# Owen-Liuyuxuan/FSNet

Measured on AMD Instinct MI355X. Metric: training samples/sec (3-frame triplets) at 192x640, ResNet-18 depth+pose, higher is better.
Workload: dtype bf16; 1 GPU; KITTI Eigen-Zhou-shaped synthetic triplets, ResNet-18 depth+pose, 192x640, bf16, batch 12/GPU, full step (fwd+loss+bwd+clip35+Adam); inputs HBM-resident, no H2D in the timed region; global_batch=12, parallelism=dp1, encoder_pass=two chains (depth and pose encoder on two streams), autotune_steps=0, hipgraph_replays=574

## Files before the change

fsnet_amd/csrc/pool_upsample.hip:

```cpp
#include "common.h"
#include "fsnet_hip_internal.h"
#include <algorithm>

namespace {

struct FsPoolPair { const void* in1; void* out1; uint8_t* idx1; const void* add1; int n0; };

template <typename T>
__global__ __launch_bounds__(256) void maxpool_fwd_kernel(const T* __restrict__ x, T* __restrict__ y,
                                                          uint8_t* __restrict__ idx, int N, int H, int W, int C,
                                                          int Ho, int Wo, FsPoolPair pr) {
  constexpr int VN = VecN<T>::N;
  const int CG = C / VN;
  const long total = (long)N * Ho * Wo * CG;
  for (long i = (long)blockIdx.x * 256 + threadIdx.x; i < total; i += (long)gridDim.x * 256) {
    int cg = (int)(i % CG); long m = i / CG;
    int wo = (int)(m % Wo); long q = m / Wo; int ho = (int)(q % Ho); long n = q / Ho;
    const T* xs = x; T* ys = y; uint8_t* is = idx;
    if (n >= pr.n0) {
      n -= pr.n0; m -= (long)pr.n0 * Ho * Wo;
      xs = reinterpret_cast<const T*>(pr.in1); ys = reinterpret_cast<T*>(pr.out1); is = pr.idx1;
    }
    float best[VN];
    int bi[VN];
#pragma unroll
    for (int j = 0; j < VN; ++j) { best[j] = -INFINITY; bi[j] = 0; }
    bool first = true;
    for (int r = 0; r < 3; ++r) {
      int h = ho * 2 - 1 + r;
      if ((unsigned)h >= (unsigned)H) continue;
      for (int s = 0; s < 3; ++s) {
        int w = wo * 2 - 1 + s;
        if ((unsigned)w >= (unsigned)W) continue;
        float v[VN];
        loadv<T>(xs + ((n * H + h) * W + w) * C + cg * VN, v);
#pragma unroll
        for (int j = 0; j < VN; ++j)
          if (first || v[j] > best[j]) { best[j] = v[j]; bi[j] = r * 3 + s; }
        first = false;
      }
    }
    storev<T>(ys + m * C + cg * VN, best);
#pragma unroll
    for (int k = 0; k < VN / 4; ++k) {
      uint32_t packed = (uint32_t)bi[4 * k] | ((uint32_t)bi[4 * k + 1] << 8) | ((uint32_t)bi[4 * k + 2] << 16) |
                        ((uint32_t)bi[4 * k + 3] << 24);
      reinterpret_cast<uint32_t*>(is + m * C + cg * VN)[k] = packed;
    }
  }
}

template <typename T>
__global__ __launch_bounds__(256) void maxpool_bwd_kernel(const T* __restrict__ dy, const uint8_t* __restrict__ idx,
                                                          const T* __restrict__ addend, T* __restrict__ dx, int N,
// ... 14 lines not shown
#pragma unroll
    for (int j = 0; j < VN; ++j) acc[j] = 0.f;
    if (ads) loadv<T>(ads + m * C + cg * VN, acc);
    for (int ho = (h - 1 + 1) / 2; ho <= (h + 1) / 2; ++ho) {
      if (ho < 0 || ho >= Ho) continue;
      int r = h - (ho * 2 - 1);
      if (r < 0 || r > 2) continue;
      for (int wo = w / 2; wo <= (w + 1) / 2; ++wo) {
        if (wo < 0 || wo >= Wo) continue;
        int s = w - (wo * 2 - 1);
        if (s < 0 || s > 2) continue;
        long mo = (n * Ho + ho) * Wo + wo;
        uint32_t packed[VN / 4];
#pragma unroll
        for (int k = 0; k < VN / 4; ++k) packed[k] = reinterpret_cast<const uint32_t*>(is + mo * C + cg * VN)[k];
        float g[VN];
        loadv<T>(dys + mo * C + cg * VN, g);
        int code = r * 3 + s;
#pragma unroll
        for (int j = 0; j < VN; ++j)
          if ((int)((packed[j >> 2] >> (8 * (j & 3))) & 0xff) == code) acc[j] += g[j];
      }
    }
    storev<T>(dxs + m * C + cg * VN, acc);
  }
}

template <typename T, int V> __device__ inline void ldc(const T* p, float* v) {
  if constexpr (V == 8) loadv<T>(p, v); else load4<T>(p, v);
}
template <typename T, int V> __device__ inline void stc(T* p, const float* v) {
  if constexpr (V == 8) storev<T>(p, v); else store4<T>(p, v);
}

template <typename T, int V>
__global__ __launch_bounds__(256) void upcat_pad_fwd_kernel(const T* __restrict__ a, const T* __restrict__ b,
                                                            T* __restrict__ out, int N, int h, int w, int Ca,
                                                            int Cb) {
  const int H = 2 * h, W = 2 * w, Hp = H + 2, Wp = W + 2, C = Ca + Cb, CG = C / V;
  const long total = (long)N * Hp * Wp * CG;
  for (long i = (long)blockIdx.x * 256 + threadIdx.x; i < total; i += (long)gridDim.x * 256) {
    int cg = (int)(i % CG); long m = i / CG;
    int wp = (int)(m % Wp); long q = m / Wp; int hp = (int)(q % Hp); long n = q / Hp;
    int hi = min(max(hp - 1, 0), H - 1), wi = min(max(wp - 1, 0), W - 1);
    int c = cg * V;
    float v[V];
    if (c < Ca) ldc<T, V>(a + ((n * h + (hi >> 1)) * w + (wi >> 1)) * Ca + c, v);
    else ldc<T, V>(b + ((n * H + hi) * W + wi) * Cb + (c - Ca), v);
    stc<T, V>(out + m * C + c, v);
  }
}

template <typename T, int V>
__device__ inline void fold_load(const T* dpad, long n, int hi, int wi, int H, int W, int C, int c, float* g) {
  const int Hp = H + 2, Wp = W + 2;
  int hs[2] = {hi + 1, 0}, ws[2] = {wi + 1, 0};
  int nh = 1, nw = 1;
  if (hi == 0) { hs[1] = 0; nh = 2; } else if (hi == H - 1) { hs[1] = H + 1; nh = 2; }
  if (wi == 0) { ws[1] = 0; nw = 2; } else if (wi == W - 1) { ws[1] = W + 1; nw = 2; }
#pragma unroll
  for (int j = 0; j < V; ++j) g[j] = 0.f;
  for (int x = 0; x < nh; ++x)
    for (int y = 0; y < nw; ++y) {
      float t[V];
      ldc<T, V>(dpad + ((n * Hp + hs[x]) * Wp + ws[y]) * C + c, t);
#pragma unroll
      for (int j = 0; j < V; ++j) g[j] += t[j];
    }
}

template <typename T, int V>
__global__ __launch_bounds__(256) void upcat_pad_bwd_kernel(const T* __restrict__ dpad, T* __restrict__ da,
                                                            T* __restrict__ db, int N, int h, int w, int Ca,
                                                            int Cb) {
  const int H = 2 * h, W = 2 * w, C = Ca + Cb;
  const int CGa = Ca / V, CGb = Cb / V;
  const long ta = (long)N * h * w * CGa, tb = (long)N * H * W * CGb;
  for (long i = (long)blockIdx.x * 256 + threadIdx.x; i < ta + tb; i += (long)gridDim.x * 256) {
    if (i < ta) {
      int cg = (int)(i % CGa); long m = i / CGa;
      int x = (int)(m % w); long q = m / w; int y = (int)(q % h); long n = q / h;
      float acc[V];
#pragma unroll
      for (int j = 0; j < V; ++j) acc[j] = 0.f;
      for (int dy = 0; dy < 2; ++dy)
        for (int dx = 0; dx < 2; ++dx) {
          float g[V];
          fold_load<T, V>(dpad, n, 2 * y + dy, 2 * x + dx, H, W, C, cg * V, g);
#pragma unroll
          for (int j = 0; j < V; ++j) acc[j] += g[j];
        }
      stc<T, V>(da + m * Ca + cg * V, acc);
    } else {
      long k = i - ta;
      int cg = (int)(k % CGb); long m = k / CGb;
      int x = (int)(m % W); long q = m / W; int y = (int)(q % H); long n = q / H;
      float g[V];
      fold_load<T, V>(dpad, n, y, x, H, W, C, Ca + cg * V, g);
      stc<T, V>(db + m * Cb + cg * V, g);
    }
  }
}

template <typename T> __device__ __forceinline__ float round_to(float v);
template <> __device__ __forceinline__ float round_to<float>(float v) { return v; }
template <> __device__ __forceinline__ float round_to<bf16>(float v) { return bf16_bits_to_f(f_to_bf16_bits(v)); }

template <typename T, int V>
__global__ __launch_bounds__(256) void upcat_pad_bwd_bn_kernel(const T* __restrict__ dpad, T* __restrict__ da,
                                                               T* __restrict__ db, int N, int h, int w, int Ca, int Cb,
                                                               const T* __restrict__ yact, const T* __restrict__ xraw,
                                                               const float* __restrict__ mean,
                                                               const float* __restrict__ invstd, double* __restrict__ sums,
                                                               const int nA) {
  const int H = 2 * h, W = 2 * w, C = Ca + Cb;
  const int CGa = Ca / V, CGb = Cb / V;
  if ((int)blockIdx.x >= nA) {
    const long tb = (long)N * H * W * CGb;
    const int bx = (int)blockIdx.x - nA, nB = (int)gridDim.x - nA;
    for (long k = (long)bx * 256 + threadIdx.x; k < tb; k += (long)nB * 256) {
      int cg = (int)(k % CGb); long m = k / CGb;
      int x = (int)(m % W); long q = m / W; int y = (int)(q % H); long n = q / H;
      float g[V];
      fold_load<T, V>(dpad, n, y, x, H, W, C, Ca + cg * V, g);
      stc<T, V>(db + m * Cb + cg * V, g);
    }
    return;
  }
  __shared__ float red[2][V][256];
  const int cg = threadIdx.x % CGa, c = cg * V;
  float mu[V], is[V], s1[V], s2[V];
#pragma unroll
  for (int j = 0; j < V; ++j) { mu[j] = mean[c + j]; is[j] = invstd[c + j]; s1[j] = 0.f; s2[j] = 0.f; }
  const long ta = (long)N * h * w * CGa;
  for (long i = (long)blockIdx.x * 256 + threadIdx.x; i < ta; i += (long)nA * 256) {
    long m = i / CGa;
    int x = (int)(m % w); long q = m / w; int y = (int)(q % h); long n = q / h;
    float acc[V], yy[V], xr[V];
    ldc<T, V>(yact + m * Ca + c, yy);
    ldc<T, V>(xraw + m * Ca + c, xr);
#pragma unroll
    for (int j = 0; j < V; ++j) acc[j] = 0.f;
    for (int dy = 0; dy < 2; ++dy)
      for (int dx = 0; dx < 2; ++dx) {
        float g[V];
        fold_load<T, V>(dpad, n, 2 * y + dy, 2 * x + dx, H, W, C, c, g);
#pragma unroll
        for (int j = 0; j < V; ++j) acc[j] += g[j];
      }
#pragma unroll
    for (int j = 0; j < V; ++j) {
      const float g = yy[j] > 0.f ? round_to<T>(acc[j]) : 0.f;
      acc[j] = g;
      s1[j] += g; s2[j] += g * (xr[j] - mu[j]) * is[j];
    }
    stc<T, V>(da + m * Ca + c, acc);
  }
#pragma unroll
  for (int j = 0; j < V; ++j) { red[0][j][threadIdx.x] = s1[j]; red[1][j][threadIdx.x] = s2[j]; }
  __syncthreads();
  const int PL = 256 / CGa;
  for (int t = threadIdx.x; t < CGa * 2 * V; t += 256) {
    const int g2 = t % CGa, kj = t / CGa, kind = kj / V, j = kj % V;
    float a = 0.f;
    for (int k = 0; k < PL; ++k) a += red[kind][j][k * CGa + g2];
    double* sl = sums + (long)(blockIdx.x % FS_STAT_SLOTS) * 2 * Ca;
    atomicAdd(sl + kind * Ca + g2 * V + j, (double)a);
  }
}

template <typename T, int VL>
__device__ __forceinline__ void channel_sum_body(const T* __restrict__ x, float* __restrict__ out, long M, int C, int Creal,
                                                 int CGB, int bx, int by, int gx) {
  __shared__ float red[VL][256];
  const int CG = C / VL;
  const int PL = 256 / CGB;
  const int cgl = threadIdx.x % CGB, pl = threadIdx.x / CGB;
  const int cg = by * CGB + cgl;
  float s[VL];
#pragma unroll
  for (int j = 0; j < VL; ++j) s[j] = 0.f;
  auto ld = [&](long m, float* v) {
    if constexpr (VL == 4) load4<T>(x + m * C + cg * 4, v);
    else loadv<T>(x + m * C + cg * VL, v);
  };
  if (cg < CG) {
    const long stride = (long)gx * PL;
    long m = (long)bx * PL + pl;
    for (; m + 3 * stride < M; m += 4 * stride) {
      float v0[VL], v1[VL], v2[VL], v3[VL];
      ld(m, v0); ld(m + stride, v1); ld(m + 2 * stride, v2); ld(m + 3 * stride, v3);
#pragma unroll
      for (int j = 0; j < VL; ++j) s[j] += (v0[j] + v1[j]) + (v2[j] + v3[j]);
// ... 77 lines not shown
  if (!dy || !dx || !idx || C % vn != 0 || N <= 0) return FS_EINVAL;
  if (dy1 && (!dx1 || !idx1 || N1 <= 0)) return FS_EINVAL;
  if (!dy1) N1 = 0;
  hipStream_t st = reinterpret_cast<hipStream_t>(stream);
  int Ho = (H + 2 - 3) / 2 + 1, Wo = (W + 2 - 3) / 2 + 1;
  const FsPoolPair pr{dy1, dx1, const_cast<uint8_t*>(idx1), addend1, dy1 ? N : 0x7fffffff};
  dim3 grid(grid_for((long)(N + N1) * H * W * (C / vn)));
  if (dtype == FS_DTYPE_BF16)
    hipLaunchKernelGGL(maxpool_bwd_kernel<bf16>, grid, dim3(256), 0, st, (const bf16*)dy, idx, (const bf16*)addend, (bf16*)dx, N + N1, H, W, C, Ho, Wo, pr);
  else if (dtype == FS_DTYPE_F32)
    hipLaunchKernelGGL(maxpool_bwd_kernel<float>, grid, dim3(256), 0, st, (const float*)dy, idx, (const float*)addend, (float*)dx, N + N1, H, W, C, Ho, Wo, pr);
  else return FS_EINVAL;
  return fs_launch_status();
}

extern "C" int fs_maxpool_bwd(const void* dy, const uint8_t* idx, const void* addend, void* dx, int N, int H, int W,
                              int C, int dtype, void* stream) {
  return fs_maxpool_bwd2(dy, idx, addend, dx, N, nullptr, nullptr, nullptr, nullptr, 0, H, W, C, dtype, stream);
}

extern "C" int fs_upcat_pad_fwd(const void* a, const void* b, void* out, int N, int h, int w, int Ca, int Cb,
                                int dtype, void* stream) {
  if (!a || !out || (Cb > 0 && !b) || Ca % 4 != 0 || Cb % 4 != 0) return FS_EINVAL;
  hipStream_t st = reinterpret_cast<hipStream_t>(stream);
  const bool wide = dtype == FS_DTYPE_BF16 && Ca % 8 == 0 && Cb % 8 == 0;
  dim3 grid(grid_for((long)N * (2 * h + 2) * (2 * w + 2) * ((Ca + Cb) / (wide ? 8 : 4))));
  if (wide)
    hipLaunchKernelGGL((upcat_pad_fwd_kernel<bf16, 8>), grid, dim3(256), 0, st, (const bf16*)a, (const bf16*)b, (bf16*)out, N, h, w, Ca, Cb);
  else if (dtype == FS_DTYPE_BF16)
    hipLaunchKernelGGL((upcat_pad_fwd_kernel<bf16, 4>), grid, dim3(256), 0, st, (const bf16*)a, (const bf16*)b, (bf16*)out, N, h, w, Ca, Cb);
  else if (dtype == FS_DTYPE_F32)
    hipLaunchKernelGGL((upcat_pad_fwd_kernel<float, 4>), grid, dim3(256), 0, st, (const float*)a, (const float*)b, (float*)out, N, h, w, Ca, Cb);
  else return FS_EINVAL;
  return fs_launch_status();
}

extern "C" int fs_upcat_pad_bwd(const void* dpad, void* da, void* db, int N, int h, int w, int Ca, int Cb, int dtype,
                                void* stream) {
  if (!dpad || !da || (Cb > 0 && !db) || Ca % 4 != 0 || Cb % 4 != 0) return FS_EINVAL;
  hipStream_t st = reinterpret_cast<hipStream_t>(stream);
  const bool wide = dtype == FS_DTYPE_BF16 && Ca % 8 == 0 && Cb % 8 == 0;
  const int V = wide ? 8 : 4;
  dim3 grid(grid_for((long)N * h * w * (Ca / V) + (long)N * 4 * h * w * (Cb / V)));
  if (wide)
    hipLaunchKernelGGL((upcat_pad_bwd_kernel<bf16, 8>), grid, dim3(256), 0, st, (const bf16*)dpad, (bf16*)da, (bf16*)db, N, h, w, Ca, Cb);
  else if (dtype == FS_DTYPE_BF16)
    hipLaunchKernelGGL((upcat_pad_bwd_kernel<bf16, 4>), grid, dim3(256), 0, st, (const bf16*)dpad, (bf16*)da, (bf16*)db, N, h, w, Ca, Cb);
  else if (dtype == FS_DTYPE_F32)
    hipLaunchKernelGGL((upcat_pad_bwd_kernel<float, 4>), grid, dim3(256), 0, st, (const float*)dpad, (float*)da, (float*)db, N, h, w, Ca, Cb);
  else return FS_EINVAL;
  return fs_launch_status();
}

extern "C" int fs_upcat_pad_bwd_bn(const void* dpad, void* da, void* db, int N, int h, int w, int Ca, int Cb, const void* y,
                                   const void* x, const float* mean, const float* invstd, double* sums, int dtype,
                                   void* stream) {
  if (!dpad || !da || (Cb > 0 && !db) || !y || !x || !mean || !invstd || !sums || Ca % 4 != 0 || Cb % 4 != 0 || Ca <= 0)
    return FS_EINVAL;
  hipStream_t st = reinterpret_cast<hipStream_t>(stream);
  const bool wide = dtype == FS_DTYPE_BF16 && Ca % 8 == 0 && Cb % 8 == 0;
  const int V = wide ? 8 : 4;
  const int CGa = Ca / V;
  if (CGa > 256 || 256 % CGa != 0) return FS_EINVAL;
  const long ta = (long)N * h * w * CGa, tb = (long)N * 4 * h * w * (Cb / V);
  const int nA = (int)std::max<long>(1, std::min<long>((ta + 511) / 512, 512));
  const int nB = Cb > 0 ? grid_for(tb) : 0;
  dim3 grid(nA + nB);
  if (wide)
    hipLaunchKernelGGL((upcat_pad_bwd_bn_kernel<bf16, 8>), grid, dim3(256), 0, st, (const bf16*)dpad, (bf16*)da, (bf16*)db, N, h, w, Ca, Cb,
                       (const bf16*)y, (const bf16*)x, mean, invstd, sums, nA);
  else if (dtype == FS_DTYPE_BF16)
    hipLaunchKernelGGL((upcat_pad_bwd_bn_kernel<bf16, 4>), grid, dim3(256), 0, st, (const bf16*)dpad, (bf16*)da, (bf16*)db, N, h, w, Ca, Cb,
                       (const bf16*)y, (const bf16*)x, mean, invstd, sums, nA);
  else if (dtype == FS_DTYPE_F32)
    hipLaunchKernelGGL((upcat_pad_bwd_bn_kernel<float, 4>), grid, dim3(256), 0, st, (const float*)dpad, (float*)da, (float*)db, N, h, w, Ca, Cb,
                       (const float*)y, (const float*)x, mean, invstd, sums, nA);
  else return FS_EINVAL;
  return fs_launch_status();
}

extern "C" int fs_channel_sum_multi(const void* const* x, float* const* out, const int64_t* M, const int32_t* C,
                                    const int32_t* Creal, int n, int dtype, void* stream) {
  if (!x || !out || !M || !C || !Creal || n < 1 || n > FS_CSUM_MAX) return FS_EINVAL;
  const int es = dtype == FS_DTYPE_BF16 ? 2 : 4;
  const int VW = 16 / es;
  CsumBatch b;
  int blocks = 0;
  bool wide = true;
  for (int i = 0; i < n; ++i) {
    if (!x[i] || !out[i] || C[i] % 4 != 0 || M[i] <= 0) return FS_EINVAL;
    wide = wide && (C[i] % VW == 0 && VW != 4);
  }
  const int VL = wide ? VW : 4;
  for (int i = 0; i < n; ++i) {
    const int CG = C[i] / VL;
    int CGB = 1;
    while (CGB < CG && CGB < 64) CGB <<= 1;
    const int PL = 256 / CGB;
    const int gx = (int)std::max<long>(1, std::min<long>((M[i] + 4L * PL - 1) / (4L * PL), 256));
    const int gy = (CG + CGB - 1) / CGB;
    b.x[i] = x[i]; b.out[i] = out[i]; b.M[i] = M[i]; b.C[i] = C[i]; b.Creal[i] = Creal[i]; b.CGB[i] = CGB; b.gx[i] = gx;
    b.start[i] = blocks;
    blocks += gx * gy;
  }
  b.start[n] = blocks; b.n = n;
  hipStream_t st = reinterpret_cast<hipStream_t>(stream);
  if (dtype == FS_DTYPE_BF16) {
    if (wide) hipLaunchKernelGGL((channel_sum_multi_kernel<bf16, 8>), dim3(blocks), dim3(256), 0, st, b);
    else hipLaunchKernelGGL((channel_sum_multi_kernel<bf16, 4>), dim3(blocks), dim3(256), 0, st, b);
  } else if (dtype == FS_DTYPE_F32) {
    hipLaunchKernelGGL((channel_sum_multi_kernel<float, 4>), dim3(blocks), dim3(256), 0, st, b);
  } else return FS_EINVAL;
  return fs_launch_status();
}

extern "C" int fs_channel_sum(const void* x, float* out, int64_t M, int C, int Creal, int dtype, void* stream) {
  if (!x || !out || C % 4 != 0 || M <= 0) return FS_EINVAL;
  hipStream_t st = reinterpret_cast<hipStream_t>(stream);
  const int es = dtype == FS_DTYPE_BF16 ? 2 : 4;
  const int VW = 16 / es;
  const bool wide = C % VW == 0 && VW != 4;
  const int VL = wide ? VW : 4;
  const int CG = C / VL;
  int CGB = 1;
  while (CGB < CG && CGB < 64) CGB <<= 1;
  const int PL = 256 / CGB;
  dim3 grid((unsigned)std::max<long>(1, std::min<long>((M + 4L * PL - 1) / (4L * PL), 256)), (CG + CGB - 1) / CGB);
  if (dtype == FS_DTYPE_BF16) {
    if (wide) hipLaunchKernelGGL((channel_sum_kernel<bf16, 8>), grid, dim3(256), 0, st, (const bf16*)x, out, (long)M, C, Creal, CGB);
// ... 7 lines not shown
```

fsnet_amd/engine/nets.py:

```python
import os
import weakref

import torch

from ..hip import ops
from ..hip.binding import raw_stream
from ..hip.conv import ConvOp, run_specs
from .runtime import RT, grad_of

STAT_SLOTS = ops.STAT_SLOTS
FOLD_BN = os.environ.get("FSNET_AMD_BN_FOLD", "1").strip().lower() not in ("0", "off", "false", "no")


class StatsPool:

    def __init__(self, device, capacity=1 << 21):
        self.buf = torch.zeros(capacity, dtype=torch.float64, device=device)
        self.off = 0
        self.high = 0
        self.dirty = False
        self.epoch = -1
        ops.register_prezero(self, StatsPool._prezero, device)

    def _prezero(self):
        self.off = 0
        self.epoch = ops.PREZERO_EPOCH[0]
        if not self.dirty:
            return []
        self.dirty = False
        return [self.buf[:self.high]]

    def reset(self):
        if self.dirty:
            self.buf[:self.high].zero_()
            self.dirty = False
        self.off = 0

    def span(self, a, b):
        if a is None or b is None or a.untyped_storage().data_ptr() != self.buf.untyped_storage().data_ptr() \
                or b.untyped_storage().data_ptr() != self.buf.untyped_storage().data_ptr():
            return None
        oa, ob = a.storage_offset(), b.storage_offset()
        if oa + a.numel() != ob:
            return None
        return self.buf[oa:ob + b.numel()]

    def take(self, C, groups=1):
        n = groups * STAT_SLOTS * 2 * C
        shape = (STAT_SLOTS, 2, C) if groups == 1 else (groups, STAT_SLOTS, 2, C)
        if self.off + n > self.buf.numel():
            return torch.zeros(shape, dtype=torch.float64, device=self.buf.device)
        v = self.buf[self.off:self.off + n].view(shape)
        self.off += n
        self.high = max(self.high, self.off)
        self.dirty = True
        return v


_PENDING_JOIN = set()
_PENDING_KEEP = []
_DEFERRED = {}
_CALLBACK_QUEUED = [None]
_ACTIVE_CHAINS = set()

# ... 985 lines not shown
            self.up1[i] = (ConvLayer(b1.sequence[0], valid_over_padded=True), b1.sequence[1])
        for s in module.scales:
            self.disp[s] = ConvLayer(module.convs[("dispconv", s)], valid_over_padded=True)
        self.unc = {s: ConvLayer(module.convs[("uncertain_logz", s)], valid_over_padded=True)
                    for s in module.scales if ("uncertain_logz", s) in module.convs}
        self.pool = None
        self._border0 = None
        self.tail_pending = False

    def forward(self, feats, train, P2=None):
        m = self.m
        dev, dt = feats[-1].device, feats[-1].dtype
        if self.pool is None or self.pool.buf.device != dev:
            self.pool = StatsPool(dev)
        self.pool.reset()
        if train:
            _check_train_bn(self.up0[4][1], "DepthDecoder")
        base_fx = getattr(m, "base_fx", None)
        if base_fx is None or P2 is None:
            P2, base_fx = None, None
        else:
            P2 = P2.detach().to(dev, torch.float32).contiguous()
        ctx = {"lv": {}, "feats": feats, "P2": P2, "base_fx": base_fx}
        outs = {}
        x = feats[-1]
        K = int(m.num_output_channels)
        aside = bool(RT.overlap and dev.type == "cuda" and RT.wgrad_streams)
        cur = _current_stream(dev) if aside else None
        ws = RT.companion_stream(dev, cur)[1] if aside else None
        put_off, used_ws = None, False

        def head(i, lv, y1p):
            cld = self.disp[i]
            opd = cld.ready(dt, dev)
            lv["logits"] = opd.forward(y1p, bias=cld.bias, out_f32=True)
            if i in self.unc:
                clu = self.unc[i]
                opu = clu.ready(dt, dev)
                lv["unc"] = ops.sigmoid_head_fwd(opu.forward(y1p, bias=clu.bias, out_f32=True))

        for i in range(4, -1, -1):
            cl0, bn0 = self.up0[i]
            op0 = cl0.ready(dt, dev)
            N, h, w, _ = x.shape
            st_a = self.pool.take(op0.Co_p) if train else None
            c0 = op0.forward(x, bias=cl0.bias, stats=st_a)
            if put_off is not None:
                ev, j, lvj, yj = put_off
                ws.wait_event(ev)
                with torch.cuda.stream(ws):
                    head(j, lvj, yj)
                put_off, used_ws = None, True
            world = _dp_stats(st_a) if train else 1
            y0 = torch.empty(N, h, w, op0.Co_p, dtype=dt, device=dev)
            s0 = ops.BnState(op0.Co_p, dev)
            ops.bn_apply(c0, st_a, bn_tensors(bn0), s0, y0, h, w, N * h * w * world, relu=True, track=train)
            skip = feats[i - 1] if (m.use_skips and i > 0) else None
            xcat = ops.upcat_pad_fwd(y0, skip)
            cl1, bn1 = self.up1[i]
            op1 = cl1.ready(dt, dev)
            H2, W2 = 2 * h, 2 * w
            st_b = self.pool.take(op1.Co_p) if train else None
            c1 = op1.forward(xcat, bias=cl1.bias, stats=st_b)
            world = _dp_stats(st_b) if train else 1
            y1p = torch.empty(N, H2 + 2, W2 + 2, op1.Co_p, dtype=dt, device=dev)
            s1 = ops.BnState(op1.Co_p, dev)
            ops.bn_apply(c1, st_b, bn_tensors(bn1), s1, y1p, H2, W2, N * H2 * W2 * world, relu=True, pad_out=True,
                         track=train)
            lv = dict(x=x, c0=c0, y0=y0, s0=s0, xcat=xcat, c1=c1, y1p=y1p, s1=s1, h=h, w=w,
                      Cs=(skip.shape[3] if skip is not None else 0))
            if i in m.scales:
                if aside and i > 0:
                    ev = torch.cuda.Event()
                    ev.record(cur)
                    put_off = (ev, i, lv, y1p)
                else:
                    head(i, lv, y1p)
            ctx["lv"][i] = lv
            x = y1p[:, 1:-1, 1:-1]
        if used_ws:
            cur.wait_stream(ws)
        sc = [i for i in range(4, -1, -1) if "logits" in ctx["lv"][i]]
        if getattr(m, "sigmoid_head", False):
            a, bq = 1.0 / float(m.max_depth), 1.0 / float(m.min_depth) - 1.0 / float(m.max_depth)
            scale = None if P2 is None else (P2[:, 0, 0] / float(base_fx)).view(-1, 1, 1, 1)
            for i in sc:
                lv = ctx["lv"][i]
                u = ops.sigmoid_head_fwd(lv["logits"])
                inv = torch.reciprocal(a + bq * u)
                depth = inv if scale is None else inv * scale
                lv["sig"] = (u, depth)
                outs[i] = (lv["logits"], depth, u)
            return outs, ctx
        if sc:
            heads = ops.depth_head_fwd_multi([ctx["lv"][i]["logits"] for i in sc], m.depth_bins, K, m.min_depth,
                                             m.max_depth, P2=P2, base_fx=base_fx)
            for i, (depth, disp) in zip(sc, heads):
                lv = ctx["lv"][i]
                outs[i] = (lv["logits"], depth, disp) + ((lv["unc"],) if "unc" in lv else ())
        return outs, ctx

    def backward(self, ctx, g_depth, g_disp, g_unc=None):
        g_unc = g_unc or {}
        m = self.m
        feats = ctx["feats"]
        dev, dt = feats[-1].device, feats[-1].dtype
        K = int(m.num_output_channels)
        gfeats = [None] * 5
        bwd_pool_reset(dev)
        chain_begins(dev)
        RT.mark("ddec.bwd.start")
# ... 133 lines not shown
```

fsnet_amd/hip/ops.py:

```python
import ctypes as C
import os

import torch

from .binding import (lib, check, stream_ptr, FsBnApplyArgs, FsBnBwdArgs, FsFlowArgs, FsMotionMaskArgs, FsPhotoArgs,
                      FsPostOptArgs, FsSmoothArgs)
from .conv import dtype_code, _timed, BN_EPS, BN_MOMENTUM, Spec, run_specs

STAT_SLOTS = 8


def _p(t):
    return t.data_ptr() if t is not None else None


def nchw_to_nhwc(a, b, cp, dtype, out=None):
    a = a.contiguous()
    N, Ca, H, W = a.shape
    Cb = 0
    if b is not None:
        b = b.contiguous()
        Cb = b.shape[1]
    if out is None:
        out = torch.empty(N, H, W, cp, dtype=dtype, device=a.device)
# ... 163 lines not shown
                     torch.empty(N, Ho, Wo, Cc, dtype=torch.uint8, device=x.device)))
    if len(xs) == 2 and xs[0].shape[1:] == xs[1].shape[1:] and xs[0].dtype == xs[1].dtype:
        x, x1 = xs
        (y, idx), (y1, idx1) = outs
        N, H, W, Cc = x.shape
        _timed("maxpool_fwd", sum(t.numel() * t.element_size() * 1.25 + o[1].numel() for t, o in zip(xs, outs)),
               lambda: check(lib.fs_maxpool_fwd2(x.data_ptr(), y.data_ptr(), idx.data_ptr(), N, x1.data_ptr(), y1.data_ptr(),
                                                 idx1.data_ptr(), x1.shape[0], H, W, Cc, dtype_code(x.dtype), stream_ptr()),
                             "maxpool_fwd"), tag=str(tuple(x.shape)) + " || " + str(tuple(x1.shape)))
        return outs
    for x, (y, idx) in zip(xs, outs):
        N, H, W, Cc = x.shape
        _timed("maxpool_fwd", x.numel() * x.element_size() * 1.25 + idx.numel(),
               lambda: check(lib.fs_maxpool_fwd(x.data_ptr(), y.data_ptr(), idx.data_ptr(), N, H, W, Cc, dtype_code(x.dtype),
                                                stream_ptr()), "maxpool_fwd"), tag=str(tuple(x.shape)))
    return outs


def maxpool_bwd(dy, idx, H, W, addend=None):
    return maxpool_bwd_multi([dy], [idx], H, W, [addend])[0]


def maxpool_bwd_multi(dys, idxs, H, W, addends):
    dxs = [torch.empty(dy.shape[0], H, W, dy.shape[3], dtype=dy.dtype, device=dy.device) for dy in dys]
    work = lambda dx, idx, ad: dx.numel() * dx.element_size() * (1.25 + (ad is not None)) + idx.numel()
    if len(dys) == 2 and dys[0].shape[1:] == dys[1].shape[1:] and dys[0].dtype == dys[1].dtype:
        dy, dy1 = dys
        Cc = dy.shape[3]
        _timed("maxpool_bwd", sum(work(dx, i, a) for dx, i, a in zip(dxs, idxs, addends)),
               lambda: check(lib.fs_maxpool_bwd2(dy.data_ptr(), idxs[0].data_ptr(), _p(addends[0]), dxs[0].data_ptr(),
                                                 dy.shape[0], dy1.data_ptr(), idxs[1].data_ptr(), _p(addends[1]),
                                                 dxs[1].data_ptr(), dy1.shape[0], H, W, Cc, dtype_code(dy.dtype),
                                                 stream_ptr()), "maxpool_bwd"),
               tag=str(tuple(dxs[0].shape)) + " || " + str(tuple(dxs[1].shape)))
        return dxs
    for dy, idx, ad, dx in zip(dys, idxs, addends, dxs):
        _timed("maxpool_bwd", work(dx, idx, ad),
               lambda: check(lib.fs_maxpool_bwd(dy.data_ptr(), idx.data_ptr(), _p(ad), dx.data_ptr(), dy.shape[0], H, W,
                                                dy.shape[3], dtype_code(dy.dtype), stream_ptr()), "maxpool_bwd"),
               tag=str(tuple(dx.shape)))
    return dxs


def upcat_pad_fwd(a, b):
    N, h, w, Ca = a.shape
    Cb = b.shape[3] if b is not None else 0
    out = torch.empty(N, 2 * h + 2, 2 * w + 2, Ca + Cb, dtype=a.dtype, device=a.device)
    _timed("upcat_pad_fwd", (a.numel() + (b.numel() if b is not None else 0) + out.numel()) * a.element_size(),
           lambda: check(lib.fs_upcat_pad_fwd(a.data_ptr(), _p(b), out.data_ptr(), N, h, w, Ca, Cb, dtype_code(a.dtype),
                                              stream_ptr()), "upcat_pad_fwd"), tag=str(tuple(out.shape)))
    return out


def upcat_pad_bwd(dpad, h, w, Ca, Cb, bn=None):
    N = dpad.shape[0]
    da = torch.empty(N, h, w, Ca, dtype=dpad.dtype, device=dpad.device)
    db = torch.empty(N, 2 * h, 2 * w, Cb, dtype=dpad.dtype, device=dpad.device) if Cb else None
    nbytes = (da.numel() + (db.numel() if db is not None else 0) + dpad.numel()) * da.element_size()
    if bn is not None:
        y, x, st, sums = bn
        assert y.is_contiguous() and x.is_contiguous() and y.shape == da.shape == x.shape and st.groups == 1
        assert sums.dtype == torch.float64 and sums.numel() == STAT_SLOTS * 2 * Ca
        _timed("upcat_pad_bwd", nbytes + 2 * da.numel() * da.element_size(),
               lambda: check(lib.fs_upcat_pad_bwd_bn(dpad.data_ptr(), da.data_ptr(), _p(db), N, h, w, Ca, Cb, y.data_ptr(),
                                                     x.data_ptr(), st.mean.data_ptr(), st.invstd.data_ptr(), sums.data_ptr(),
                                                     dtype_code(dpad.dtype), stream_ptr()), "upcat_pad_bwd_bn"),
               tag=str(tuple(dpad.shape)) + " bn")
        return da, db
    _timed("upcat_pad_bwd", nbytes,
           lambda: check(lib.fs_upcat_pad_bwd(dpad.data_ptr(), da.data_ptr(), _p(db), N, h, w, Ca, Cb,
                                              dtype_code(dpad.dtype), stream_ptr()), "upcat_pad_bwd"),
           tag=str(tuple(dpad.shape)))
    return da, db


def channel_sum(x, out, creal):
    Cc = x.shape[-1]
    M = x.numel() // Cc
    _timed("channel_sum", x.numel() * x.element_size(),
           lambda: check(lib.fs_channel_sum(x.data_ptr(), out.data_ptr(), M, Cc, creal, dtype_code(x.dtype),
                                            stream_ptr()), "channel_sum"), tag=str(tuple(x.shape)))


def channel_sum_multi(items):
    items = list(items)
    if len(items) == 1:
        return channel_sum(*items[0])
    for i in range(0, len(items), 16):
        chunk = items[i:i + 16]
        n = len(chunk)
        code = dtype_code(chunk[0][0].dtype)
        assert all(dtype_code(x.dtype) == code for x, _, _ in chunk)
        xs = (C.c_void_p * n)(*[x.data_ptr() for x, _, _ in chunk])
        outs = (C.c_void_p * n)(*[o.data_ptr() for _, o, _ in chunk])
        Ms = (C.c_int64 * n)(*[x.numel() // x.shape[-1] for x, _, _ in chunk])
        Cs = (C.c_int32 * n)(*[x.shape[-1] for x, _, _ in chunk])
        Cr = (C.c_int32 * n)(*[int(cr) for _, _, cr in chunk])
        _timed("channel_sum", sum(x.numel() * x.element_size() for x, _, _ in chunk),
               lambda: check(lib.fs_channel_sum_multi(xs, outs, Ms, Cs, Cr, n, code, stream_ptr()), "channel_sum_multi"),
               tag="%d tensors" % n)


def depth_head_fwd(logits, bins, K, min_depth, max_depth):
    N, H, W, Cl = logits.shape
    depth = torch.empty(N, 1, H, W, dtype=torch.float32, device=logits.device)
    disp = torch.empty(N, 1, H, W, dtype=torch.float32, device=logits.device)
    check(lib.fs_depth_head_fwd(logits.data_ptr(), bins.data_ptr(), depth.data_ptr(), disp.data_ptr(), N * H * W, K,
                                Cl, float(min_depth), float(max_depth), stream_ptr()), "depth_head_fwd")
    return depth, disp


def depth_head_bwd(logits, bins, d_depth, d_disp, K, min_depth, max_depth, dtype):
    N, H, W, Cl = logits.shape
    dl = torch.empty(N, H, W, Cl, dtype=dtype, device=logits.device)
    check(lib.fs_depth_head_bwd(logits.data_ptr(), bins.data_ptr(), _p(d_depth), _p(d_disp), dl.data_ptr(),
# ... 657 lines not shown
```

fsnet_amd/hip/signatures.py:

```python
import ctypes as C

P = C.c_void_p
I = C.c_int
L = C.c_int64
F = C.c_float
D = C.c_double

SIGNATURES = {
    "fs_abi_version": (C.c_int, []),
    "fs_target_arch": (C.c_char_p, []),
    "fs_debug_timestamp": (C.c_int, [P, P]),
    "fs_capture_position": (C.c_int, [P, P]),
    "fs_conv_igemm": (C.c_int, [P, I, P]),
    "fs_conv_igemm2": (C.c_int, [P, P, I, P]),
    "fs_conv3x3_halo2": (C.c_int, [P, P, I, P]),
    "fs_conv3x3_halo2_plan": (C.c_int, [P, P, I, P]),
    "fs_conv3x3_s2d": (C.c_int, [P, I, P]),
    "fs_conv3x3_s2d2": (C.c_int, [P, P, I, P]),
    "fs_conv_stem2": (C.c_int, [P, P, I, P]),
    "fs_conv_wgrad2": (C.c_int, [P, P, I, P]),
    "fs_conv_wgrad2_plan": (C.c_int, [P, P, I, P]),
    "fs_bn_apply2": (C.c_int, [P, P, I, P]),
    "fs_bn_bwd_reduce2": (C.c_int, [P, P, I, P]),
    "fs_bn_bwd_apply2": (C.c_int, [P, P, I, P]),
    "fs_maxpool_fwd2": (C.c_int, [P, P, P, I, P, P, P, I, I, I, I, I, P]),
    "fs_maxpool_bwd2": (C.c_int, [P, P, P, P, I, P, P, P, P, I, I, I, I, I, P]),
    "fs_conv3x3_halo": (C.c_int, [P, I, P]),
    "fs_conv3x3_halo_plan": (C.c_int, [P, I, P]),
    "fs_conv1x1": (C.c_int, [P, I, P]),
    "fs_conv_stem": (C.c_int, [P, I, P]),
    "fs_conv_wgrad": (C.c_int, [P, I, P]),
    "fs_conv_wgrad_plan": (C.c_int, [P, I, P]),
    "fs_pack_weights": (C.c_int, [P, P, I, I, I, I, I, I, L, I, I, P]),
    "fs_sigmoid_head_fwd": (C.c_int, [P, P, L, I, P]),
    "fs_sigmoid_head_bwd": (C.c_int, [P, P, P, L, I, I, P]),
    "fs_distill_fwd": (C.c_int, [P, P, P, L, P, P]),
    "fs_distill_bwd": (C.c_int, [P, P, P, L, P, P, P, P]),
    "fs_resize_linear": (C.c_int, [P, P, I, I, I, I, I, P]),
    "fs_depth_eval": (C.c_int, [P, P, I, I, I, I, I, P, P, P]),
    "fs_depth_eval_masked": (C.c_int, [P, P, P, I, I, I, I, I, F, F, I, P, P, P]),
    "fs_lidar_mei_depth": (C.c_int, [P, P, L, P, P, I, I, I, P, P, P, L, P]),
    "fs_lidar_mei_depth_workspace_bytes": (C.c_int64, [I, I, I]),
    "fs_lidar_pinhole_depth": (C.c_int, [P, P, L, P, I, I, I, P, P, L, P]),
    "fs_lidar_pinhole_depth_workspace_bytes": (C.c_int64, [I, I, I]),
    "fs_postopt": (C.c_int, [P, P]),
    "fs_postopt_workspace_bytes": (C.c_int64, [I, I, I, I]),
    "fs_optflow_farneback": (C.c_int, [P, P]),
    "fs_optflow_workspace_bytes": (C.c_int64, [P]),
    "fs_optflow_level_image": (C.c_int, [P, I, P, P]),
    "fs_motion_mask": (C.c_int, [P, P]),
    "fs_augment_masks": (C.c_int, [P, P, P, P, P, I, I, I, I, I, P]),
    "fs_copy_multi": (C.c_int, [P, P, P, I, P]),
    "fs_zero_multi": (C.c_int, [P, P, I, P]),
    "fs_pack_tile_blocks": (C.c_int64, [C.c_int, C.c_int, C.c_int, C.c_int]),
    "fs_pack_weights_multi": (C.c_int, [P, I, L, I, P]),
    "fs_nchw_to_nhwc": (C.c_int, [P, P, P, I, I, I, I, I, I, I, P]),
    "fs_bn_apply": (C.c_int, [P, I, P]),
    "fs_bn_finalize": (C.c_int, [P, P, P, P]),
    "fs_bn_bwd_reduce": (C.c_int, [P, I, P]),
    "fs_bn_bwd_apply": (C.c_int, [P, I, P]),
    "fs_maxpool_fwd": (C.c_int, [P, P, P, I, I, I, I, I, P]),
    "fs_maxpool_bwd": (C.c_int, [P, P, P, P, I, I, I, I, I, P]),
    "fs_upcat_pad_fwd": (C.c_int, [P, P, P, I, I, I, I, I, I, P]),
    "fs_upcat_pad_bwd": (C.c_int, [P, P, P, I, I, I, I, I, I, P]),
    "fs_upcat_pad_bwd_bn": (C.c_int, [P, P, P, I, I, I, I, I, P, P, P, P, P, I, P]),
    "fs_channel_sum": (C.c_int, [P, P, L, I, I, I, P]),
    "fs_channel_sum_multi": (C.c_int, [P, P, P, P, P, I, I, P]),
    "fs_depth_head_fwd": (C.c_int, [P, P, P, P, L, I, I, F, F, P]),
    "fs_depth_head_bwd": (C.c_int, [P, P, P, P, P, L, I, I, F, F, I, P]),
    "fs_depth_head_fwd_multi": (C.c_int, [P, P, I, I, F, F, P]),
    "fs_depth_head_bwd_multi": (C.c_int, [P, P, I, I, F, F, I, P]),
    "fs_pose_tail_fwd": (C.c_int, [P, P, P, P, I, I, I, I, I, F, P]),
    "fs_pose_tail_bwd": (C.c_int, [P, P, P, I, I, I, I, I, F, I, P]),
    "fs_photo_setup": (C.c_int, [P, P, P, P, I, P, I, P]),
    "fs_mei_lut": (C.c_int, [P, I, I, F, F, F, F, D, D, D, P]),
    "fs_mei_stage_mask": (C.c_int, [P, P, P, I, I, I, P]),
    "fs_mei_points": (C.c_int, [P, P, P, I, I, I, P]),
    "fs_photo_identity": (C.c_int, [P, P]),
    "fs_photo_fused_fwd": (C.c_int, [P, P]),
    "fs_photo_fused_bwd": (C.c_int, [P, P]),
    "fs_photo_fused_bwd_tiles": (C.c_int64, [I, I]),
    "fs_photo_pose_grad": (C.c_int, [P, P, P, P, I, I, I, P]),
    "fs_augment_frames": (C.c_int, [P, P]),
    "fs_resize_frames": (C.c_int, [P, P]),
    "fs_color_pyramid": (C.c_int, [P, P, I, I, I, I, I, P]),
    "fs_smooth_mean": (C.c_int, [P, P]),
    "fs_smooth_fwd": (C.c_int, [P, P]),
    "fs_smooth_bwd": (C.c_int, [P, P]),
    "fs_loss_finalize": (C.c_int, [P, P, P, P, P, P, P]),
    "fs_sumsq": (C.c_int, [P, L, P, P, P]),
    "fs_counter_incr": (C.c_int, [P, P]),
    "fs_adam_step": (C.c_int, [P, P, P, P, L, F, F, F, F, F, I, F, P, F, P, P, P]),
}


def declare(lib):
    for name, (res, args) in SIGNATURES.items():
        fn = getattr(lib, name)
        fn.restype = res
        fn.argtypes = args
```

include/fsnet_hip.h:

```cpp
#ifndef FSNET_HIP_H
#define FSNET_HIP_H
#include <stdint.h>

#ifdef __cplusplus
extern "C" {
#endif

#define FS_OK 0
#define FS_EINVAL 1
#define FS_ELAUNCH 2

#define FS_DTYPE_F32 0
#define FS_DTYPE_BF16 1

#define FS_STAT_SLOTS 8

#define FS_ABI_VERSION 15
int fs_abi_version(void);
const char* fs_target_arch(void);
int fs_debug_timestamp(void* slot, void* stream);
int fs_capture_position(void* stream, unsigned long long* token);

typedef struct FsConvArgs {
  const void* src;
// ... 221 lines not shown
  const double* stats;  const double* stats2;
  const float* gamma;   const float* beta;
  const float* gamma2;  const float* beta2;
  float* running_mean;  float* running_var;
  float* running_mean2; float* running_var2;
  int64_t* num_batches_tracked; int64_t* num_batches_tracked2;
  float* save_mean;  float* save_invstd;
  float* save_mean2; float* save_invstd2;
  double count;
  float eps, momentum;
  int64_t yN, yH, yW;
  int32_t M, C, H, W;
  int32_t relu, pad_out;
  int32_t groups;
  void* pool_y; uint8_t* pool_idx;
} FsBnApplyArgs;
int fs_bn_apply(const FsBnApplyArgs* args, int dtype, void* stream);
int fs_bn_apply2(const FsBnApplyArgs* a0, const FsBnApplyArgs* a1, int dtype, void* stream);
int fs_bn_finalize(const FsBnApplyArgs* args, float* scale, float* shift, void* stream);

typedef struct FsBnBwdArgs {
  const void* dout; const void* y; const void* x;
  void* dx; void* g_out;
  double* sums; const double* sums_local;
  const float* gamma; const float* save_mean; const float* save_invstd;
  float* dgamma; float* dbeta;
  double count;
  int64_t gN, gH, gW;
  int64_t yN, yH, yW;
  int32_t M, C, H, W;
  int32_t relu, fold;
  int32_t groups;
  const void* pool_dy; const uint8_t* pool_idx; const float* beta;
} FsBnBwdArgs;
int fs_bn_bwd_reduce(const FsBnBwdArgs* args, int dtype, void* stream);
int fs_bn_bwd_apply(const FsBnBwdArgs* args, int dtype, void* stream);
int fs_bn_bwd_reduce2(const FsBnBwdArgs* a0, const FsBnBwdArgs* a1, int dtype, void* stream);
int fs_bn_bwd_apply2(const FsBnBwdArgs* a0, const FsBnBwdArgs* a1, int dtype, void* stream);

int fs_maxpool_fwd(const void* x, void* y, uint8_t* idx, int N, int H, int W, int C, int dtype, void* stream);
int fs_maxpool_bwd(const void* dy, const uint8_t* idx, const void* addend, void* dx, int N, int H, int W, int C,
                   int dtype, void* stream);
int fs_maxpool_fwd2(const void* x, void* y, uint8_t* idx, int N, const void* x1, void* y1, uint8_t* idx1, int N1, int H,
                    int W, int C, int dtype, void* stream);
int fs_maxpool_bwd2(const void* dy, const uint8_t* idx, const void* addend, void* dx, int N, const void* dy1,
                    const uint8_t* idx1, const void* addend1, void* dx1, int N1, int H, int W, int C, int dtype,
                    void* stream);
int fs_upcat_pad_fwd(const void* a, const void* b, void* out, int N, int h, int w, int Ca, int Cb, int dtype,
                     void* stream);
int fs_upcat_pad_bwd(const void* dpad, void* da, void* db, int N, int h, int w, int Ca, int Cb, int dtype,
                     void* stream);
int fs_upcat_pad_bwd_bn(const void* dpad, void* da, void* db, int N, int h, int w, int Ca, int Cb, const void* y,
                        const void* x, const float* mean, const float* invstd, double* sums, int dtype, void* stream);
int fs_channel_sum(const void* x, float* out, int64_t M, int C, int Creal, int dtype, void* stream);
int fs_channel_sum_multi(const void* const* x, float* const* out, const int64_t* M, const int32_t* C, const int32_t* Creal,
                         int n, int dtype, void* stream);

int fs_depth_head_fwd(const float* logits, const float* bins, float* depth, float* disp, int64_t M, int K, int Cl,
                      float min_depth, float max_depth, void* stream);
int fs_depth_head_bwd(const float* logits, const float* bins, const float* d_depth, const float* d_disp,
                      void* dlogits, int64_t M, int K, int Cl, float min_depth, float max_depth, int dtype,
                      void* stream);

#define FS_HEAD_MAX 4
typedef struct FsHeadBatch {
  const float* logits[4];
  float* depth[4];
  float* disp[4];
  const float* d_depth[4];
  const float* d_disp[4];
  void* dlogits[4];
  int64_t M[4];
  int32_t n;
  int32_t nimg;
  const float* P2;
  float base_fx;
  int32_t reserved;
} FsHeadBatch;
int fs_depth_head_fwd_multi(const FsHeadBatch* batch, const float* bins, int K, int Cl, float min_depth,
                            float max_depth, void* stream);
int fs_depth_head_bwd_multi(const FsHeadBatch* batch, const float* bins, int K, int Cl, float min_depth,
                            float max_depth, int dtype, void* stream);

int fs_pose_tail_fwd(const float* x, float* axisangle, float* translation, float* T, int B, int hw, int Cx,
                     int nframes, int invert, float scale, void* stream);
int fs_pose_tail_bwd(const float* x, const float* dT, void* dx, int B, int hw, int Cx, int nframes, int invert,
                     float scale, int dtype, void* stream);

typedef struct FsPhotoArgs {
  const float* img0;
  const float* img_src[2];
  const double* patched_mask;
  const float* depth[4];
  const float* geo;
  float* pred;
  uint8_t* ov;
  float* ident;
  uint8_t* sel;
  double* loss_sums;
  double* mask_sum;
  float* d_depth[4];
  float* dP;
  const double* gout;
  int32_t dh[4], dw[4];
  int32_t B, H, W, S;
  int32_t noise_seed;
// ... 52 lines not shown
```

Measured before the change: 2274 samples/s.

## Fuse decoder BN-apply+ReLU into upsample-concat-pad and derive activations in backward

```diff
diff --git a/fsnet_amd/csrc/pool_upsample.hip b/fsnet_amd/csrc/pool_upsample.hip
--- a/fsnet_amd/csrc/pool_upsample.hip
+++ b/fsnet_amd/csrc/pool_upsample.hip
@@ -1,5 +1,6 @@
 #include "common.h"
 #include "fsnet_hip_internal.h"
+#include "conv_pro.h"
 #include <algorithm>
 
 namespace {
@@ -120,6 +121,49 @@
 }
 
 template <typename T, int V>
+__global__ __launch_bounds__(256) void upcat_pad_fwd_bn_kernel(const FsConvArgs p, const T* __restrict__ a,
+                                                               const T* __restrict__ b, T* __restrict__ out, int N, int h,
+                                                               int w, int Ca, int Cb) {
+  extern __shared__ float upcat_tab[];
+  const int H = 2 * h, W = 2 * w, Hp = H + 2, Wp = W + 2, C = Ca + Cb, CG = C / V;
+  const long total = (long)N * Hp * Wp * CG;
+  const bool small = total < (1L << 31);
+  auto fetch = [&](long i, float* v, int& c, long& m) {
+    int cg, wp, hp; long n;
+    if (small) {
+      const unsigned u = (unsigned)i, q = u / (unsigned)CG, q2 = q / (unsigned)Wp, q3 = q2 / (unsigned)Hp;
+      cg = (int)(u - q * CG); m = q; wp = (int)(q - q2 * Wp); hp = (int)(q2 - q3 * Hp); n = q3;
+    } else {
+      cg = (int)(i % CG); m = i / CG;
+      wp = (int)(m % Wp); const long q = m / Wp; hp = (int)(q % Hp); n = q / Hp;
+    }
+    const int hi = min(max(hp - 1, 0), H - 1), wi = min(max(wp - 1, 0), W - 1);
+    c = cg * V;
+    if (c < Ca) ldc<T, V>(a + ((n * h + (hi >> 1)) * w + (wi >> 1)) * Ca + c, v);
+    else ldc<T, V>(b + ((n * H + hi) * W + wi) * Cb + (c - Ca), v);
+  };
+  const long stride = (long)gridDim.x * 256;
+  long i = (long)blockIdx.x * 256 + threadIdx.x;
+  float nv[V]; int nc = 0; long nm = 0;
+  if (i < total) fetch(i, nv, nc, nm);
+  pro_build_table<1>(p, upcat_tab, 0, threadIdx.x, 256);
+  if (blockIdx.x == 0) pro_block0<1>(p, threadIdx.x, 256);
+  __syncthreads();
+  for (; i < total; i += stride) {
+    float v[V];
+    const int c = nc; const long m = nm;
+#pragma unroll
+    for (int j = 0; j < V; ++j) v[j] = nv[j];
+    if (i + stride < total) fetch(i + stride, nv, nc, nm);
+    if (c < Ca) {
+#pragma unroll
+      for (int j = 0; j < V; ++j) v[j] = fmaxf(v[j] * upcat_tab[c + j] + upcat_tab[Ca + c + j], 0.f);
+    }
+    stc<T, V>(out + m * C + c, v);
+  }
+}
+
+template <typename T, int V>
 __device__ inline void fold_load(const T* dpad, long n, int hi, int wi, int H, int W, int C, int c, float* g) {
   const int Hp = H + 2, Wp = W + 2;
   int hs[2] = {hi + 1, 0}, ws[2] = {wi + 1, 0};
@@ -174,13 +218,14 @@
 template <> __device__ __forceinline__ float round_to<float>(float v) { return v; }
 template <> __device__ __forceinline__ float round_to<bf16>(float v) { return bf16_bits_to_f(f_to_bf16_bits(v)); }
 
-template <typename T, int V>
+template <typename T, int V, bool DER>
 __global__ __launch_bounds__(256) void upcat_pad_bwd_bn_kernel(const T* __restrict__ dpad, T* __restrict__ da,
                                                                T* __restrict__ db, int N, int h, int w, int Ca, int Cb,
                                                                const T* __restrict__ yact, const T* __restrict__ xraw,
                                                                const float* __restrict__ mean,
                                                                const float* __restrict__ invstd, double* __restrict__ sums,
-                                                               const int nA) {
+                                                               const int nA, const float* __restrict__ msc,
+                                                               const float* __restrict__ msh) {
   const int H = 2 * h, W = 2 * w, C = Ca + Cb;
   const int CGa = Ca / V, CGb = Cb / V;
   if ((int)blockIdx.x >= nA) {
@@ -197,16 +242,23 @@
   }
   __shared__ float red[2][V][256];
   const int cg = threadIdx.x % CGa, c = cg * V;
-  float mu[V], is[V], s1[V], s2[V];
-#pragma unroll
-  for (int j = 0; j < V; ++j) { mu[j] = mean[c + j]; is[j] = invstd[c + j]; s1[j] = 0.f; s2[j] = 0.f; }
+  float mu[V], is[V], s1[V], s2[V], ks[V], kh[V];
+#pragma unroll
+  for (int j = 0; j < V; ++j) {
+    mu[j] = mean[c + j]; is[j] = invstd[c + j]; s1[j] = 0.f; s2[j] = 0.f;
+    ks[j] = DER ? msc[c + j] : 0.f; kh[j] = DER ? msh[c + j] : 0.f;
+  }
   const long ta = (long)N * h * w * CGa;
   for (long i = (long)blockIdx.x * 256 + threadIdx.x; i < ta; i += (long)nA * 256) {
     long m = i / CGa;
     int x = (int)(m % w); long q = m / w; int y = (int)(q % h); long n = q / h;
     float acc[V], yy[V], xr[V];
-    ldc<T, V>(yact + m * Ca + c, yy);
     ldc<T, V>(xraw + m * Ca + c, xr);
+    if constexpr (!DER) ldc<T, V>(yact + m * Ca + c, yy);
+    else {
+#pragma unroll
+      for (int j = 0; j < V; ++j) yy[j] = xr[j] * ks[j] + kh[j];
+    }
 #pragma unroll
     for (int j = 0; j < V; ++j) acc[j] = 0.f;
     for (int dy = 0; dy < 2; ++dy)
@@ -390,11 +442,13 @@
   return fs_launch_status();
 }
 
-extern "C" int fs_upcat_pad_bwd_bn(const void* dpad, void* da, void* db, int N, int h, int w, int Ca, int Cb, const void* y,
-                                   const void* x, const float* mean, const float* invstd, double* sums, int dtype,
-                                   void* stream) {
-  if (!dpad || !da || (Cb > 0 && !db) || !y || !x || !mean || !invstd || !sums || Ca % 4 != 0 || Cb % 4 != 0 || Ca <= 0)
+namespace {
+int upcat_pad_bwd_bn_launch(const void* dpad, void* da, void* db, int N, int h, int w, int Ca, int Cb, const void* y,
+                            const void* x, const float* mean, const float* invstd, const float* scale, const float* shift,
+                            double* sums, int dtype, void* stream) {
+  if (!dpad || !da || (Cb > 0 && !db) || !x || !mean || !invstd || !sums || Ca % 4 != 0 || Cb % 4 != 0 || Ca <= 0)
     return FS_EINVAL;
+  if (!y && (!scale || !shift)) return FS_EINVAL;
   hipStream_t st = reinterpret_cast<hipStream_t>(stream);
   const bool wide = dtype == FS_DTYPE_BF16 && Ca % 8 == 0 && Cb % 8 == 0;
   const int V = wide ? 8 : 4;
@@ -404,15 +458,58 @@
   const int nA = (int)std::max<long>(1, std::min<long>((ta + 511) / 512, 512));
   const int nB = Cb > 0 ? grid_for(tb) : 0;
   dim3 grid(nA + nB);
+#define UPCAT_BWD_BN(T, V, DER)                                                                                        \
+  hipLaunchKernelGGL((upcat_pad_bwd_bn_kernel<T, V, DER>), grid, dim3(256), 0, st, (const T*)dpad, (T*)da, (T*)db, N, h, w, \
+                     Ca, Cb, (const T*)y, (const T*)x, mean, invstd, sums, nA, scale, shift)
+  if (wide) { if (y) UPCAT_BWD_BN(bf16, 8, false); else UPCAT_BWD_BN(bf16, 8, true); }
+  else if (dtype == FS_DTYPE_BF16) { if (y) UPCAT_BWD_BN(bf16, 4, false); else UPCAT_BWD_BN(bf16, 4, true); }
+  else if (dtype == FS_DTYPE_F32) { if (y) UPCAT_BWD_BN(float, 4, false); else UPCAT_BWD_BN(float, 4, true); }
+#undef UPCAT_BWD_BN
+  else return FS_EINVAL;
+  return fs_launch_status();
+}
+}
+
+extern "C" int fs_upcat_pad_bwd_bn(const void* dpad, void* da, void* db, int N, int h, int w, int Ca, int Cb, const void* y,
+                                   const void* x, const float* mean, const float* invstd, double* sums, int dtype,
+                                   void* stream) {
+  if (!y) return FS_EINVAL;
+  return upcat_pad_bwd_bn_launch(dpad, da, db, N, h, w, Ca, Cb, y, x, mean, invstd, nullptr, nullptr, sums, dtype, stream);
+}
+
+extern "C" int fs_upcat_pad_bwd_bn_derived(const void* dpad, void* da, void* db, int N, int h, int w, int Ca, int Cb,
+                                           const void* x, const float* mean, const float* invstd, const float* scale,
+                                           const float* shift, double* sums, int dtype, void* stream) {
+  return upcat_pad_bwd_bn_launch(dpad, da, db, N, h, w, Ca, Cb, nullptr, x, mean, invstd, scale, shift, sums, dtype, stream);
+}
+
+extern "C" int fs_upcat_pad_fwd_bn(const FsBnApplyArgs* bn, float* scale, float* shift, const void* b, void* out, int N,
+                                   int h, int w, int Cb, int dtype, void* stream) {
+  if (!bn || !bn->x || !bn->stats || !bn->gamma || !bn->beta || !bn->save_mean || !bn->save_invstd || !scale || !shift || !out)
+    return FS_EINVAL;
+  const int Ca = bn->C;
+  if (bn->groups > 1 || !(bn->count > 0.0) || N <= 0 || h <= 0 || w <= 0 || (long)N * h * w != (long)bn->M) return FS_EINVAL;
+  if ((Cb > 0 && !b) || Cb < 0 || Ca <= 0 || Ca > 512 || Ca % 4 != 0 || Cb % 4 != 0) return FS_EINVAL;
+  if ((bn->running_mean == nullptr) != (bn->running_var == nullptr)) return FS_EINVAL;
+  FsConvArgs p{};
+  p.N = N; p.Cs = Ca;
+  p.pro_mode = 1; p.pro_relu = 1;
+  p.pro_stats = bn->stats; p.pro_gamma = bn->gamma; p.pro_beta = bn->beta;
+  p.pro_mean = bn->save_mean; p.pro_invstd = bn->save_invstd; p.pro_save_a = scale; p.pro_save_b = shift;
+  p.pro_running_mean = bn->running_mean; p.pro_running_var = bn->running_var; p.pro_nbt = bn->num_batches_tracked;
+  p.pro_count = bn->count; p.pro_eps = bn->eps; p.pro_momentum = bn->momentum;
+  hipStream_t st = reinterpret_cast<hipStream_t>(stream);
+  const bool wide = dtype == FS_DTYPE_BF16 && Ca % 8 == 0 && Cb % 8 == 0;
+  const long total = (long)N * (2 * h + 2) * (2 * w + 2) * ((Ca + Cb) / (wide ? 8 : 4));
+  dim3 grid((unsigned)std::max<long>(1, std::min<long>((total + 1023) / 1024, 1024)));
+  const unsigned lds = 2u * Ca * sizeof(float);
+  const void* a = bn->x;
   if (wide)
-    hipLaunchKernelGGL((upcat_pad_bwd_bn_kernel<bf16, 8>), grid, dim3(256), 0, st, (const bf16*)dpad, (bf16*)da, (bf16*)db, N, h, w, Ca, Cb,
-                       (const bf16*)y, (const bf16*)x, mean, invstd, sums, nA);
+    hipLaunchKernelGGL((upcat_pad_fwd_bn_kernel<bf16, 8>), grid, dim3(256), lds, st, p, (const bf16*)a, (const bf16*)b, (bf16*)out, N, h, w, Ca, Cb);
   else if (dtype == FS_DTYPE_BF16)
-    hipLaunchKernelGGL((upcat_pad_bwd_bn_kernel<bf16, 4>), grid, dim3(256), 0, st, (const bf16*)dpad, (bf16*)da, (bf16*)db, N, h, w, Ca, Cb,
-                       (const bf16*)y, (const bf16*)x, mean, invstd, sums, nA);
+    hipLaunchKernelGGL((upcat_pad_fwd_bn_kernel<bf16, 4>), grid, dim3(256), lds, st, p, (const bf16*)a, (const bf16*)b, (bf16*)out, N, h, w, Ca, Cb);
   else if (dtype == FS_DTYPE_F32)
-    hipLaunchKernelGGL((upcat_pad_bwd_bn_kernel<float, 4>), grid, dim3(256), 0, st, (const float*)dpad, (float*)da, (float*)db, N, h, w, Ca, Cb,
-                       (const float*)y, (const float*)x, mean, invstd, sums, nA);
+    hipLaunchKernelGGL((upcat_pad_fwd_bn_kernel<float, 4>), grid, dim3(256), lds, st, p, (const float*)a, (const float*)b, (float*)out, N, h, w, Ca, Cb);
   else return FS_EINVAL;
   return fs_launch_status();
 }
diff --git a/fsnet_amd/engine/nets.py b/fsnet_amd/engine/nets.py
--- a/fsnet_amd/engine/nets.py
+++ b/fsnet_amd/engine/nets.py
@@ -10,6 +10,7 @@
 
 STAT_SLOTS = ops.STAT_SLOTS
 FOLD_BN = os.environ.get("FSNET_AMD_BN_FOLD", "1").strip().lower() not in ("0", "off", "false", "no")
+FOLD_DECODER_BN = os.environ.get("FSNET_AMD_DECODER_FOLD", "1").strip().lower() not in ("0", "off", "false", "no")
 
 
 class StatsPool:
@@ -1101,11 +1102,16 @@
                     head(j, lvj, yj)
                 put_off, used_ws = None, True
             world = _dp_stats(st_a) if train else 1
-            y0 = torch.empty(N, h, w, op0.Co_p, dtype=dt, device=dev)
-            s0 = ops.BnState(op0.Co_p, dev)
-            ops.bn_apply(c0, st_a, bn_tensors(bn0), s0, y0, h, w, N * h * w * world, relu=True, track=train)
             skip = feats[i - 1] if (m.use_skips and i > 0) else None
-            xcat = ops.upcat_pad_fwd(y0, skip)
+            if train and FOLD_DECODER_BN and op0.Co_p <= 512:
+                y0 = None
+                s0 = ops.BnState(op0.Co_p, dev, affine=True)
+                xcat = ops.upcat_pad_fwd_bn(c0, st_a, bn_tensors(bn0), s0, skip, N * h * w * world, track=True)
+            else:
+                y0 = torch.empty(N, h, w, op0.Co_p, dtype=dt, device=dev)
+                s0 = ops.BnState(op0.Co_p, dev)
+                ops.bn_apply(c0, st_a, bn_tensors(bn0), s0, y0, h, w, N * h * w * world, relu=True, track=train)
+                xcat = ops.upcat_pad_fwd(y0, skip)
             cl1, bn1 = self.up1[i]
             op1 = cl1.ready(dt, dev)
             H2, W2 = 2 * h, 2 * w
diff --git a/fsnet_amd/hip/ops.py b/fsnet_amd/hip/ops.py
--- a/fsnet_amd/hip/ops.py
+++ b/fsnet_amd/hip/ops.py
@@ -239,6 +239,30 @@
     return out
 
 
+def upcat_pad_fwd_bn(c, stats, bn, st, b, count, track=True):
+    N, h, w, Ca = c.shape
+    Cb = b.shape[3] if b is not None else 0
+    assert c.is_contiguous() and (b is None or b.is_contiguous()) and stats is not None
+    assert st.groups == 1 and st.scale is not None
+    out = torch.empty(N, 2 * h + 2, 2 * w + 2, Ca + Cb, dtype=c.dtype, device=c.device)
+    a = FsBnApplyArgs()
+    a.x, a.stats = c.data_ptr(), stats.data_ptr()
+    a.gamma, a.beta = bn["weight"].data_ptr(), bn["bias"].data_ptr()
+    if track:
+        a.running_mean, a.running_var = bn["running_mean"].data_ptr(), bn["running_var"].data_ptr()
+        a.num_batches_tracked = bn["num_batches_tracked"].data_ptr()
+    a.save_mean, a.save_invstd = st.mean.data_ptr(), st.invstd.data_ptr()
+    st.count = float(count)
+    a.count, a.eps, a.momentum = float(count), BN_EPS, BN_MOMENTUM
+    a.M, a.C, a.H, a.W = N * h * w, Ca, h, w
+    a.relu = 1
+    _timed("upcat_pad_fwd", (c.numel() + (b.numel() if b is not None else 0) + out.numel()) * c.element_size(),
+           lambda: check(lib.fs_upcat_pad_fwd_bn(C.byref(a), st.scale.data_ptr(), st.shift.data_ptr(), _p(b), out.data_ptr(),
+                                                 N, h, w, Cb, dtype_code(c.dtype), stream_ptr()), "upcat_pad_fwd_bn"),
+           tag=str(tuple(out.shape)) + " bn")
+    return out
+
+
 def upcat_pad_bwd(dpad, h, w, Ca, Cb, bn=None):
     N = dpad.shape[0]
     da = torch.empty(N, h, w, Ca, dtype=dpad.dtype, device=dpad.device)
@@ -246,8 +270,18 @@
     nbytes = (da.numel() + (db.numel() if db is not None else 0) + dpad.numel()) * da.element_size()
     if bn is not None:
         y, x, st, sums = bn
-        assert y.is_contiguous() and x.is_contiguous() and y.shape == da.shape == x.shape and st.groups == 1
+        assert x.is_contiguous() and da.shape == x.shape and st.groups == 1
         assert sums.dtype == torch.float64 and sums.numel() == STAT_SLOTS * 2 * Ca
+        if y is None:
+            assert st.scale is not None
+            _timed("upcat_pad_bwd", nbytes + da.numel() * da.element_size(),
+                   lambda: check(lib.fs_upcat_pad_bwd_bn_derived(dpad.data_ptr(), da.data_ptr(), _p(db), N, h, w, Ca, Cb,
+                                                                 x.data_ptr(), st.mean.data_ptr(), st.invstd.data_ptr(),
+                                                                 st.scale.data_ptr(), st.shift.data_ptr(), sums.data_ptr(),
+                                                                 dtype_code(dpad.dtype), stream_ptr()),
+                                 "upcat_pad_bwd_bn_derived"), tag=str(tuple(dpad.shape)) + " bn")
+            return da, db
+        assert y.is_contiguous() and y.shape == da.shape
         _timed("upcat_pad_bwd", nbytes + 2 * da.numel() * da.element_size(),
                lambda: check(lib.fs_upcat_pad_bwd_bn(dpad.data_ptr(), da.data_ptr(), _p(db), N, h, w, Ca, Cb, y.data_ptr(),
                                                      x.data_ptr(), st.mean.data_ptr(), st.invstd.data_ptr(), sums.data_ptr(),
diff --git a/fsnet_amd/hip/signatures.py b/fsnet_amd/hip/signatures.py
--- a/fsnet_amd/hip/signatures.py
+++ b/fsnet_amd/hip/signatures.py
@@ -64,6 +64,8 @@
     "fs_upcat_pad_fwd": (C.c_int, [P, P, P, I, I, I, I, I, I, P]),
     "fs_upcat_pad_bwd": (C.c_int, [P, P, P, I, I, I, I, I, I, P]),
     "fs_upcat_pad_bwd_bn": (C.c_int, [P, P, P, I, I, I, I, I, P, P, P, P, P, I, P]),
+    "fs_upcat_pad_bwd_bn_derived": (C.c_int, [P, P, P, I, I, I, I, I, P, P, P, P, P, P, I, P]),
+    "fs_upcat_pad_fwd_bn": (C.c_int, [P, P, P, P, P, I, I, I, I, I, P]),
     "fs_channel_sum": (C.c_int, [P, P, L, I, I, I, P]),
     "fs_channel_sum_multi": (C.c_int, [P, P, P, P, P, I, I, P]),
     "fs_depth_head_fwd": (C.c_int, [P, P, P, P, L, I, I, F, F, P]),
diff --git a/include/fsnet_hip.h b/include/fsnet_hip.h
--- a/include/fsnet_hip.h
+++ b/include/fsnet_hip.h
@@ -297,6 +297,11 @@
                      void* stream);
 int fs_upcat_pad_bwd_bn(const void* dpad, void* da, void* db, int N, int h, int w, int Ca, int Cb, const void* y,
                         const void* x, const float* mean, const float* invstd, double* sums, int dtype, void* stream);
+int fs_upcat_pad_bwd_bn_derived(const void* dpad, void* da, void* db, int N, int h, int w, int Ca, int Cb, const void* x,
+                                const float* mean, const float* invstd, const float* scale, const float* shift,
+                                double* sums, int dtype, void* stream);
+int fs_upcat_pad_fwd_bn(const FsBnApplyArgs* bn, float* scale, float* shift, const void* b, void* out, int N, int h, int w,
+                        int Cb, int dtype, void* stream);
 int fs_channel_sum(const void* x, float* out, int64_t M, int C, int Creal, int dtype, void* stream);
 int fs_channel_sum_multi(const void* const* x, float* const* out, const int64_t* M, const int32_t* C, const int32_t* Creal,
                          int n, int dtype, void* stream);
```

After: 2280 samples/s, median of 6. No clear change (+0.3%).
